# JacobYoung115/VisualSLAM

Measured on AMD Instinct MI355X. Metric: frames/sec @1080p (Harris + DoG keypoint detection), higher is better.
Workload: dtype u8

## Files before the change

visualslam_amd/csrc/kernels_aux.hip.h:

```cpp
#pragma once
#include <hip/hip_runtime.h>

#include "kernels_generic.hip.h"
#include "kernels_localize.hip.h"

namespace vslam {

__global__ __launch_bounds__(256) void k_resize_linear2x_slide(const uint8_t* __restrict__ src, size_t sstep, size_t sframe,
                                                                uint8_t* __restrict__ dst, size_t dframe, int dpitch,
                                                                int rows, int cols, int seg) {
    const int k = blockIdx.x * 256 + threadIdx.x;
    if (4 * k >= cols) return;
    const bool whole = 4 * k + 3 < cols;
    const int m0 = blockIdx.y * seg, m1 = min(m0 + seg, rows);
    const uint8_t* s = src + blockIdx.z * sframe;
    uint8_t* d = dst + blockIdx.z * dframe + 8 * k;
    const int xl = max(4 * k - 1, 0), xr = min(4 * k + 4, cols - 1);
    auto hrow = [&](int m, uint32_t (&X)[4], uint32_t (&Y)[4]) {
        const uint8_t* r = s + (size_t)min(max(m, 0), rows - 1) * sstep;
        uint32_t w;
        if (whole)
            __builtin_memcpy(&w, r + 4 * k, 4);
        else
            w = (uint32_t)r[4 * k] | ((uint32_t)r[min(4 * k + 1, cols - 1)] << 8) | ((uint32_t)r[min(4 * k + 2, cols - 1)] << 16) |
                ((uint32_t)r[cols - 1] << 24);
        const uint32_t s0 = r[xl], s5 = r[xr];
        const uint32_t P = __builtin_amdgcn_perm(w, w, 0x0c010c00);
        const uint32_t Q = __builtin_amdgcn_perm(w, w, 0x0c030c02);
        const uint32_t Qm = __builtin_amdgcn_perm(w, w, 0x0c020c01);
        const uint32_t Pm = s0 | ((w & 0xffu) << 16);
        const uint32_t Qp = (w >> 24) | (s5 << 16);
        const uint32_t P3 = P + (P << 1), Q3 = Q + (Q << 1);
        const uint32_t A[4] = {Pm + P3, P3 + Qm, Qm + Q3, Q3 + Qp};
#pragma unroll
        for (int i = 0; i < 4; ++i) {
            X[i] = pk_lshr_u16(A[i], 2);
            Y[i] = pk_lshr_u16(A[i] + (A[i] << 1), 2);
        }
    };
    auto emit = [&](int dy, const uint32_t (&U)[4], const uint32_t (&V)[4]) {
        uint32_t v[4];
#pragma unroll
        for (int i = 0; i < 4; ++i) v[i] = pk_lshr_u16(U[i] + V[i] + 0x00020002u, 2);
        *reinterpret_cast<uint2*>(d + (size_t)dy * dpitch) = make_uint2(v[0] | (v[1] << 8), v[2] | (v[3] << 8));
    };
    uint32_t Xp[4], Yp[4], Xc[4], Yc[4];
    hrow(m0 - 1, Xp, Yp);
    hrow(m0, Xc, Yc);
    for (int m = m0; m < m1; ++m) {
        uint32_t Xn[4], Yn[4];
        hrow(m + 1, Xn, Yn);
        emit(2 * m, Xp, Yc);
        emit(2 * m + 1, Yc, Xn);
#pragma unroll
        for (int i = 0; i < 4; ++i) Xp[i] = Xc[i], Xc[i] = Xn[i], Yc[i] = Yn[i];
    }
}

__global__ __launch_bounds__(256) void k_resize_nearest_half_v4(const uint8_t* __restrict__ src, size_t sframe, int spitch,
                                                                 uint8_t* __restrict__ dst, size_t dframe, int dpitch,
                                                                 int rows, int drows, int dcols) {
    const int k = blockIdx.x * 256 + threadIdx.x;
    const int y = blockIdx.y;
    if (4 * k >= dcols) return;
    const int sy = min(2 * y, rows - 1);
    const uint2 w = *reinterpret_cast<const uint2*>(src + blockIdx.z * sframe + (size_t)sy * spitch + 8 * k);
    *reinterpret_cast<uint32_t*>(dst + blockIdx.z * dframe + (size_t)y * dpitch + 4 * k) =
        even_bytes(w.x, w.y);
}

constexpr int EXT_SPAN = 768;
constexpr int EXT_PITCH = EXT_SPAN + 16;

template <bool LOC>
__global__ __launch_bounds__(256) void k_extrema_w3(const uint8_t* __restrict__ pyr, size_t pframe, ExtGeom g, int o,
                                                     unsigned long long* __restrict__ bits,
                                                     unsigned long long* __restrict__ lflags, size_t bframe, int li0, int li_step) {
    constexpr int NROW = LOC ? 13 : 10;
    __shared__ __attribute__((aligned(16))) uint8_t srow[NROW * EXT_PITCH + 16];
    __shared__ uint2 queue[LOC ? 768 : 1];
    __shared__ uint8_t qkeep[LOC ? 768 : 1];
    const int li = li0 + (int)blockIdx.y * li_step, f = blockIdx.z;
    const int rows = g.rows[o], cols = g.cols[o], pitch = g.pitch[o];
    const uint32_t P = (uint32_t)rows * (uint32_t)pitch;
    const uint8_t* dog = pyr + f * pframe + g.oct_off[o] + (size_t)VSLAM_NUM_LEVELS * P;
    const int ya = max(3 * li - 1, 0), yb = 3 * li;
    const int yc = min(3 * li + 1, rows - 1);
    const int c0 = blockIdx.x * EXT_SPAN - 16;
    const int wave = __builtin_amdgcn_readfirstlane(threadIdx.x >> 6), lane = threadIdx.x & 63;
    const int cpiece = c0 + 16 * lane;
    const bool piece_ok = lane < EXT_PITCH / 16 && cpiece >= 0 && cpiece < cols;
#pragma unroll
    for (int i = 0; i < (NROW + 3) / 4; ++i) {
        const int rl = wave + 4 * i;
        if (rl < NROW) {
            const int lev = rl < 10 ? (rl >> 1) : rl - 9, y = rl < 10 ? ((rl & 1) ? yb : ya) : yc;
            const uint8_t* rowp = dog + (ptrdiff_t)(int)((uint32_t)lev * P + (uint32_t)y * (uint32_t)pitch + (uint32_t)c0);
            if (piece_ok)
                *reinterpret_cast<uint4*>(srow + rl * EXT_PITCH + 16 * lane) =
                    *reinterpret_cast<const uint4*>(rowp + (uint32_t)(16 * lane));
        }
    }
    if (blockIdx.x == 0 && threadIdx.x < 10)
        srow[threadIdx.x * EXT_PITCH + 15] = dog[(threadIdx.x >> 1) * P + (uint32_t)((threadIdx.x & 1) ? yb : ya) * (uint32_t)pitch];
    __syncthreads();
    const int lc = g.lat_cols[o], wpr = g.wpr[o], lr = g.lat_rows[o];
    const int lj = blockIdx.x * 256 + threadIdx.x;
    bool cand[3] = {false, false, false}, listed[3] = {false, false, false};
    unsigned long long wcand[3], wlist[3];
    const unsigned long long owns = __builtin_amdgcn_ballot_w64(lj < lc);
    const int xa = 3 * (int)threadIdx.x - 1 + 16;
    uint32_t self[5];
    uint32_t up[5], left[5];
    {
        const uint32_t s = xa & 3;
        const uint32_t sel = 0x0c000c00u | s | ((s + 1) << 16);
        uint32_t mn[5], mx[5];
#pragma unroll
        for (int l = 0; l < 5; ++l) {
            uint32_t off = (uint32_t)(xa & ~3) + (uint32_t)(2 * l * EXT_PITCH);
            if (l) asm volatile("" : "+v"(off));
            const uint32_t* q0 = reinterpret_cast<const uint32_t*>(srow + off);
            const uint32_t* q1 = q0 + EXT_PITCH / 4;
            const uint32_t v0 = __builtin_amdgcn_perm(q0[1], q0[0], sel), v1 = __builtin_amdgcn_perm(q1[1], q1[0], sel);
            const uint32_t lo = pk_min_u16(v0, v1), hi = pk_max_u16(v0, v1);
            mn[l] = min(lo & 0xffffu, lo >> 16);
            mx[l] = max(hi & 0xffffu, hi >> 16);
            self[l] = v1 >> 16;
            if (LOC) up[l] = v0 >> 16, left[l] = v1 & 0xffffu;
        }
#pragma unroll
        for (int L = 1; L <= 3; ++L) {
            const uint32_t lo = min(mn[L - 1], min(mn[L], mn[L + 1])), hi = max(mx[L - 1], max(mx[L], mx[L + 1]));
            wcand[L - 1] = (__builtin_amdgcn_ballot_w64(self[L] == lo) | __builtin_amdgcn_ballot_w64(self[L] == hi)) & owns;
            if (LOC) cand[L - 1] = lj < lc && (self[L] == lo || self[L] == hi);
            else wlist[L - 1] = wcand[L - 1] & __builtin_amdgcn_ballot_w64((int)self[L] >= g.min_contrast);
        }
    }
// ... 110 lines not shown
```

visualslam_amd/csrc/vslam_ctx.h:

```cpp
#pragma once
#include <hip/hip_runtime.h>

#include <cstdint>
#include <cstdlib>
#include <deque>
#include <map>
#include <set>
#include <string>
#include <tuple>
#include <utility>
#include <vector>

#include "../../include/vslam.h"

#ifdef VSLAM_DIAGNOSTICS
#define VSLAM_DIAG_ENV(name) std::getenv(name)
#else
#define VSLAM_DIAG_ENV(name) (static_cast<const char*>(nullptr))
#endif

struct StreamTuner {
    static constexpr int K = 3;
    static constexpr int M = K + 1;
    hipStream_t cand[K][2] = {};
    hipEvent_t t0[M] = {}, t1[M] = {};
    int measured = 0;
    int measuring = -1;
    bool enabled = false;
    bool done = false;
    int chosen = 0;
    unsigned long long key = 0;
    int calls = 0, resets = 0;
};

struct JoinWatch {
    static constexpr int RING = 4, NEED = 3;
    hipEvent_t t0[RING] = {}, tm[RING] = {}, t1[RING] = {};
    bool live[RING] = {};
    int head = 0;
    int recording = -1;
    int calls = 0;
    int n_meas = 0;
    float lag[NEED] = {}, best_total = 0.0f;
    float level_best[3] = {0.0f, 0.0f, 0.0f};
    int level = 1;
    int trial_from = -1;
    unsigned long long key = 0;
    int restarts = 0;
    bool done = false, disabled = false, pinned = false;
    float last_lag_frac = -1.0f;
    hipStream_t pair[2][2] = {};
};

struct vslam_ctx {
    int device = 0;
    hipStream_t stream = nullptr;
    bool own_stream = false;
    std::string err;
    char* ws = nullptr;
    size_t ws_cap = 0;
    std::map<std::tuple<int, uint64_t, int>, void*> tables;
    bool mx = false;
    bool f32_fused = false;
    bool orient_scalar_form = false;
    static constexpr int kAux = 3;
    hipStream_t aux[kAux] = {nullptr, nullptr, nullptr};
    hipEvent_t ev_fork = nullptr, ev_join[kAux] = {nullptr, nullptr, nullptr}, ev_oct[VSLAM_MAX_OCTAVES] = {};
    int prio_lo = 0;
    int prio_dev_lo = 0;
    StreamTuner tuner;
    JoinWatch watch;
    hipEvent_t ev_phase = nullptr;
    bool phase_marked = false;
    hipEvent_t ev_up2 = nullptr;
    hipEvent_t ev_chunk = nullptr;
    hipEvent_t ev_pack = nullptr;
    bool pack_pending = false;
    hipEvent_t ev_list0 = nullptr, ev_edge = nullptr;
    hipEvent_t ev_or_fork = nullptr, ev_or_join[2] = {nullptr, nullptr};
    std::vector<std::pair<size_t, void*>> block_cache;
    std::set<const void*> lds_raised;
    float* loc_lut = nullptr;
    uint8_t* dump = nullptr;
    std::string timing_name;
    int launch_tag = -1;
    int timing_tag = -1;
    std::deque<std::pair<hipEvent_t, hipEvent_t>> timing_ev;
    size_t timing_used = 0;
};

static inline int fail(vslam_ctx* c, int code, const std::string& msg) {
    if (c) c->err = msg;
    return code;
}

#define HIPCHK(ctx, expr)                                                                        \
    do {                                                                                         \
        hipError_t e_ = (expr);                                                                  \
        if (e_ != hipSuccess)                                                                    \
            return fail(ctx, e_ == hipErrorOutOfMemory ? VSLAM_ERR_NOMEM : VSLAM_ERR_HIP,        \
                        std::string(#expr) + ": " + hipGetErrorString(e_));                     \
    } while (0)

#define ARGCHK(ctx, cond, msg) \
    if (!(cond)) return fail(ctx, VSLAM_ERR_INVALID, msg)
#define TRY(expr)              \
    do {                       \
        int rc_ = (expr);      \
        if (rc_) return rc_;   \
    } while (0)

static inline int bind_device(vslam_ctx* c) {
    if (!c) return VSLAM_ERR_INVALID;
    HIPCHK(c, hipSetDevice(c->device));
    return VSLAM_OK;
}

namespace vslam {
void sched_init_from_env(vslam_ctx* c);
void sched_destroy(vslam_ctx* c);
int sched_ensure_aux(vslam_ctx* c);
int sched_watch_before_call(vslam_ctx* c, unsigned long long key, bool eligible, bool capturing);
int sched_tuner_before_call(vslam_ctx* c, unsigned long long key, bool eligible);
int sched_tuner_after_call(vslam_ctx* c);
std::pair<hipEvent_t, hipEvent_t>* timing_slot(vslam_ctx* c);
}

struct TimedScope {
    vslam_ctx* c;
    std::pair<hipEvent_t, hipEvent_t>* ev;
    hipStream_t st;
    TimedScope(vslam_ctx* ctx, const char* name, int tag = -1, hipStream_t stream = nullptr)
        : c(ctx), ev(!ctx->timing_name.empty() && ctx->timing_name == name && (ctx->timing_tag < 0 || ctx->timing_tag == tag) ? vslam::timing_slot(ctx) : nullptr),
          st(stream ? stream : ctx->stream) {
        if (ev) (void)hipEventRecord(ev->first, st);
    }
    ~TimedScope() {
        if (ev) (void)hipEventRecord(ev->second, st);
    }
};
```

visualslam_amd/csrc/vslam_hip.hip:

```cpp
#include <hip/hip_runtime.h>

#include <algorithm>
#include <cstdio>
#include <cstdlib>
#include <cstring>
#include <deque>
#include <functional>
#include <map>
#include <string>
#include <set>
#include <memory>
#include <vector>

#include "../../include/vslam.h"
#include "kernels_generic.hip.h"
#include "kernels_pyramid.hip.h"
#include "kernels_strip.hip.h"
#include "kernels_hdiff.hip.h"
#include "kernels_aux.hip.h"
#include "kernels_harris_strip.hip.h"
#include "kernels_orient.hip.h"
#include "kernels_orient_batch.hip.h"
#include "kernels_orient_pk.hip.h"
#include "kernels_compact.hip.h"
// ... 442 lines not shown
}


template <class CFG>
static int enqueue_pyr_octave(vslam_ctx* c, double sigma0, int o, const OctPlan& pl, const OctIO& io) {
    const PyrTaps<CFG>* taps;
    TRY(get_table(c, kTableTile, sigma0, o, "octave kernel", sizeof(PyrTaps<CFG>), [&](void* host) -> int {
        const uint16_t* tp[6];
        tap_pointers(pl.taps, tp);
        pyr_pack_taps<CFG>(tp, *static_cast<PyrTaps<CFG>*>(host));
        return VSLAM_OK;
    }, &taps));
    TRY(raise_dyn_lds(c, reinterpret_cast<const void*>(&k_pyr_octave<CFG>)));
    const dim3 grid((io.cols + CFG::TW - 1) / CFG::TW, (io.rows + CFG::TH - 1) / CFG::TH, io.nf);
    LAUNCH_ON(c, "k_pyr_octave", o, c->stream, CFG::LDS_BYTES, k_pyr_octave<CFG>, grid, dim3(CFG::NT), io.base, io.bframe, io.oct, io.pframe, io.rows,
              io.cols, io.pitch, taps, io.next_base, io.nframe, io.nrows, io.ncols, io.npitch);
    return VSLAM_OK;
}

static int enqueue_pyr_octave_mx(vslam_ctx* c, double sigma0, int o, const OctPlan& pl, const OctIO& io, const MxScan* scan, int up2_step = 0) {
    const void* table;
    TRY(get_table(c, kTableMx, sigma0, o, "matrix-core octave kernel", mx_taps_bytes(pl.mx), [&](void* host) -> int {
        const uint16_t* tp[6];
        tap_pointers(pl.taps, tp);
        if (!mx_pack(pl.mx, tp, host)) return fail(c, VSLAM_ERR_UNSUPPORTED, "matrix-core octave kernel: a tap exceeds 127");
        HIPCHK(c, mx_prepare(pl.mx));
        return VSLAM_OK;
    }, &table));
    hipError_t e;
    {
        TimedScope ts(c, "k_pyr_octave_mx", o);
        e = mx_launch(pl.mx, c->stream, table, io, scan, up2_step);
    }
    HIPCHK(c, e);
    return VSLAM_OK;
}

static int mark_phase(vslam_ctx* c) {
    if (!c->ev_phase) HIPCHK(c, hipEventCreateWithFlags(&c->ev_phase, hipEventDisableTiming));
    HIPCHK(c, hipEventRecord(c->ev_phase, c->stream));
    c->phase_marked = true;
    return VSLAM_OK;
}

static int dog_side_gate(const std::vector<OctPlan>& plans, int nf) {
    int gate = -1;
    if (nf >= 32)
        for (int o = 0; o < (int)plans.size(); ++o)
            if (plans[o].path == OctPath::Tile0 || plans[o].path == OctPath::Tile1) gate = o;
    return gate;
}

static DenseGeom dense_geom(const vslam_batch_layout& L, int o, int min_contrast, int nf) {
    DenseGeom g;
    g.rows = L.rows[o], g.cols = L.cols[o], g.pitch = L.pitch[o];
    g.wpr = (g.cols + 63) / 64;
    g.min_contrast = min_contrast;
    g.P = (unsigned int)((size_t)g.rows * g.pitch);
    g.dog_off = (unsigned int)(L.octave_offset[o] + (size_t)VSLAM_NUM_LEVELS * g.P);
    const long waves_per_rowseg = 4L * (((g.cols + 3) / 4 + 255) / 256) * nf;
    const long segs_wanted = std::max<long>(1, 8192 / waves_per_rowseg);
    g.seg = (int)std::min<long>(XD_SEG_MAX, std::max<long>(4, (g.rows + segs_wanted - 1) / segs_wanted));
    return g;
}

namespace {
struct DogOut {
    uint8_t* pyr;
    size_t pframe;
    unsigned long long* bits = nullptr;
    bool do_extrema = false;
    vslam_point* points = nullptr;
    unsigned int* counts = nullptr;
};

struct DogRun {
    hipStream_t side = nullptr;
    hipStream_t up = nullptr;
    std::function<int(int)> after_list;
    std::function<int(int)> after_octave;
    bool later_chunk = false;
    bool bases_are_scratch = false;
};
}

static int enqueue_octave_scan(vslam_ctx* c, const vslam_params& p, const vslam_batch_layout& L, const ExtGeom& g, const DogScratch& s,
                               const MxScan* fused, int o, int o_done, int nf, const DogOut& out, const DogRun& run) {
    uint8_t* const pyr = out.pyr;
    const size_t pframe = out.pframe;
    unsigned long long* const bits = out.bits;
    const hipStream_t side = run.side;
    if (out.do_extrema && L.lat_rows[o] > 0 && L.lat_cols[o] > 0) {
        hipStream_t es = c->stream;
        if (side) {
            HIPCHK(c, hipStreamWaitEvent(side, c->ev_oct[o_done], 0));
            es = side;
        }
        if (p.extrema_dense) {
            const DenseGeom dg = dense_geom(L, o, p.min_contrast, nf);
            hipLaunchKernelGGL(k_extrema_dense, dim3(((dg.cols + 3) / 4 + 255) / 256, (dg.rows + dg.seg - 1) / dg.seg, nf), dim3(256), 0, es,
                               pyr, pframe, dg, bits ? bits + L.bits_offset[o] : nullptr, s.lflags + L.bits_offset[o], L.bits_frame_words);
        } else if (fused) {
            {
                TimedScope ts(c, "k_extrema_pack", o, es);
                HIPCHK(c, mx_launch_pack(es, *fused, L.rows[o], L.lat_words[o], nf, bits ? bits + L.bits_offset[o] : nullptr, s.lflags + L.bits_offset[o],
                                         L.bits_frame_words, kMxStripRows));
            }
            const int sr = kMxStripRows;
            const int n_straddle = (L.lat_rows[o] - 1) / sr;
            TimedScope ts(c, "k_extrema_w3", o, es);
            if (n_straddle > 0)
                hipLaunchKernelGGL(k_extrema_w3<false>, dim3((L.lat_words[o] + 3) / 4, n_straddle, nf), dim3(256), 0, es, pyr, pframe, g, o, bits, s.lflags,
                                   L.bits_frame_words, sr, sr);
            if (es != c->stream) {
                HIPCHK(c, hipEventRecord(c->ev_pack, es));
                c->pack_pending = true;
            }
        } else if (p.extrema_window == 3) {
            const dim3 eg((L.lat_words[o] + 3) / 4, L.lat_rows[o], nf);
            if (p.localize)
                LAUNCH_ON(c, "k_extrema_w3", o, es, 0, k_extrema_w3<true>, eg, dim3(256), pyr, pframe, g, o, bits, s.lflags, L.bits_frame_words, 0, 1);
            else
                LAUNCH_ON(c, "k_extrema_w3", o, es, 0, k_extrema_w3<false>, eg, dim3(256), pyr, pframe, g, o, bits, s.lflags, L.bits_frame_words, 0, 1);
        } else
            hipLaunchKernelGGL(k_extrema, dim3((L.lat_cols[o] + 255) / 256, L.lat_rows[o], nf * 3), dim3(256), 0, es, pyr,
                               pframe, g, o, bits, s.lflags, L.bits_frame_words);
        HIPCHK(c, hipGetLastError());
    }
    if (out.do_extrema && out.points && out.counts) {
        StreamSwap sw(c, side ? side : c->stream);
        const size_t entries = (size_t)3 * L.lat_rows[o] * L.lat_words[o];
        if (p.extrema_dense) {
            DenseDogEntries ent{s.lflags + L.bits_offset[o], L.bits_frame_words, pyr, pframe, dense_geom(L, o, p.min_contrast, nf), o, out.points};
            TRY(enqueue_compaction(c, ent, entries, nf, s.cws, p.dog_cap, out.counts, o > 0 ? 1 : 0));
        } else {
            DogEntries ent{s.lflags, L.bits_frame_words, pyr, pframe, g, o, o + 1, out.points};
            TRY(enqueue_compaction(c, ent, entries, nf, s.cws, p.dog_cap, out.counts, o > 0 ? 1 : 0));
        }
        if (run.after_list) TRY(run.after_list(o));
    }
    return VSLAM_OK;
}

static int enqueue_dog(vslam_ctx* c, const vslam_params& p, const vslam_batch_layout& L, const std::vector<OctPlan>& plans, const uint8_t* frames,
                       size_t fstep, size_t fframe, int nf, DogScratch& s, const DogOut& out, const DogRun& run = DogRun()) {
    const hipStream_t side = run.side, up = run.up;
    const int gate = (side && p.localize) ? dog_side_gate(plans, nf) : -1;
    ExtGeom g;
    if (p.localize) TRY(ensure_loc_lut(c));
    fill_geom(c, p, L, g);
    const bool up2_fused = c->mx && run.bases_are_scratch && L.n_octaves > 0 && L.rows[0] == 2 * p.rows && L.cols[0] == 2 * p.cols && fstep <= 0x7fffffff &&
                           mx_up2_supported(plans[0].mx);
    const int nf_a = (!up2_fused && side && up && nf >= 64) ? nf / 2 : nf;
    if (!up2_fused)
        LAUNCH(c, "k_resize_linear2x_slide", k_resize_linear2x_slide, dim3(((p.cols + 3) / 4 + 255) / 256, (p.rows + 15) / 16, nf_a), dim3(256),
               frames, fstep, fframe, s.bases + s.base_off[0], s.bases_frame, L.pitch[0], p.rows, p.cols, 16);
    if (nf_a < nf) {
        if (run.later_chunk) HIPCHK(c, hipStreamWaitEvent(up, c->ev_chunk, 0));
        StreamSwap sw(c, up);
        LAUNCH(c, "k_resize_linear2x_slide", k_resize_linear2x_slide, dim3(((p.cols + 3) / 4 + 255) / 256, (p.rows + 15) / 16, nf - nf_a), dim3(256),
               frames + (size_t)nf_a * fframe, fstep, fframe, s.bases + s.base_off[0] + (size_t)nf_a * s.bases_frame, s.bases_frame, L.pitch[0],
               p.rows, p.cols, 16);
        HIPCHK(c, hipEventRecord(c->ev_up2, c->stream));
    }
    bool fused[VSLAM_MAX_OCTAVES] = {};
    if (run.later_chunk && c->pack_pending) {
        HIPCHK(c, hipStreamWaitEvent(c->stream, c->ev_pack, 0));
        c->pack_pending = false;
    }
    MxScan scan[VSLAM_MAX_OCTAVES] = {};
    struct TagReset {
        vslam_ctx* c;
        ~TagReset() { c->launch_tag = -1; }
    } tag_reset{c};
    for (int o = 0; o < L.n_octaves; ++o) {
        c->launch_tag = o;
        const int rows = L.rows[o], cols = L.cols[o], pitch = L.pitch[o];
        const size_t P = (size_t)rows * pitch;
        const OctPlan& pl = plans[o];
        const bool has_next = o + 1 < L.n_octaves;
        const bool fuse_next = has_next && pl.path != OctPath::Generic;
        OctIO io{s.bases + s.base_off[o], s.bases_frame, out.pyr + L.octave_offset[o], out.pframe, rows, cols, pitch, nf,
                 fuse_next ? s.bases + s.base_off[o + 1] : nullptr, s.bases_frame, has_next ? L.rows[o + 1] : 0, has_next ? L.cols[o + 1] : 0,
                 has_next ? L.pitch[o + 1] : 0};
        if (o == 0 && up2_fused) io.base = frames, io.bframe = fframe;
        const int shape = (long)((cols + 255) / 256) * ((rows + 31) / 32) <= (long)((cols + 127) / 128) * ((rows + 63) / 64) ? 1 : 0;
        fused[o] = c->mx && s.sitemap && out.do_extrema && !p.localize && !p.extrema_dense && p.extrema_window == 3 && L.lat_rows[o] > 0 &&
                   L.lat_cols[o] > 0 && mx_scan_supported(pl.mx);
        if (fused[o])
            scan[o] = MxScan{s.sitemap + s.site_off[o], s.site_frame, L.lat_rows[o], L.lat_cols[o], s.site_pitch[o], p.min_contrast,
                             s.colmap + s.col_off[o], s.col_frame, mx_seams(cols)};
        auto tiled = [&](int f_lo, int n) -> int {
            const OctIO part = io.frames(f_lo, n);
            if (c->mx && pl.mx) {
                MxScan sc = scan[o];
                if (fused[o]) sc.sitemap += (size_t)f_lo * s.site_frame, sc.colmap += (size_t)f_lo * s.col_frame;
                return enqueue_pyr_octave_mx(c, p.sigma0, o, pl, part, fused[o] ? &sc : nullptr, o == 0 && up2_fused ? (int)fstep : 0);
            }
            if (pl.path == OctPath::Tile0)
                return shape == 1 ? enqueue_pyr_octave<PyrCfgOct0W>(c, p.sigma0, o, pl, part) : enqueue_pyr_octave<PyrCfgOct0>(c, p.sigma0, o, pl, part);
            return shape == 1 ? enqueue_pyr_octave<PyrCfgOct1W>(c, p.sigma0, o, pl, part) : enqueue_pyr_octave<PyrCfgOct1>(c, p.sigma0, o, pl, part);
        };
        const bool is_tiled = pl.path == OctPath::Tile0 || pl.path == OctPath::Tile1 || (c->mx && pl.mx != 0);
        if (o == 0 && nf_a < nf && !is_tiled) HIPCHK(c, hipStreamWaitEvent(c->stream, c->ev_up2, 0));
        if (is_tiled && o == 0 && nf_a < nf) {
            TRY(tiled(0, nf_a));
            HIPCHK(c, hipStreamWaitEvent(c->stream, c->ev_up2, 0));
            TRY(tiled(nf_a, nf - nf_a));
        } else if (is_tiled)
            TRY(tiled(0, nf));
        else if (pl.path == OctPath::Strip)
            TRY(enqueue_strip_octave(c, p.sigma0, o, pl, io, s.h));
        else {
            for (int l = 0; l < VSLAM_NUM_LEVELS; ++l)
                TRY(enqueue_blur(c, io.base, (size_t)pitch, s.bases_frame, io.oct + (size_t)l * P, (size_t)pitch, out.pframe, s.h, rows,
                                 cols, nf, pl.ks[l], pl.sg[l]));
            LAUNCH(c, "k_dog5", k_dog5, dim3((unsigned)((P + 255) / 256), 1, nf), dim3(256), io.oct,
                   io.oct + (size_t)VSLAM_NUM_LEVELS * P, P, out.pframe);
        }
        if (has_next && !fuse_next)
            LAUNCH(c, "k_resize_nearest_half_v4", k_resize_nearest_half_v4, dim3((L.cols[o + 1] / 4 + 256) / 256, L.rows[o + 1], nf),
                   dim3(256), io.oct + (size_t)3 * P, out.pframe, pitch, s.bases + s.base_off[o + 1], s.bases_frame, L.pitch[o + 1], rows,
                   L.rows[o + 1], L.cols[o + 1]);
        if (side) HIPCHK(c, hipEventRecord(c->ev_oct[o], c->stream));
        if (o == 0) TRY(mark_phase(c));
        if (run.after_octave) TRY(run.after_octave(o));
        if (o < gate) continue;
        for (int oo = (o == gate ? 0 : o); oo <= o; ++oo) TRY(enqueue_octave_scan(c, p, L, g, s, fused[oo] ? &scan[oo] : nullptr, oo, o, nf, out, run));
    }
    if (side && up) HIPCHK(c, hipEventRecord(c->ev_chunk, c->stream));
    return VSLAM_OK;
}

static size_t harris_flag_words(int rows, int cols) { return (size_t)rows * ((cols + HS_STRIP_W - 1) / HS_STRIP_W) * 4; }

static int enqueue_harris(vslam_ctx* c, const uint8_t* frames, size_t fframe, int rows, int cols, int nf, float k,
                          float* resp, uint8_t* mask, float* nms2, unsigned long long* hflags, vslam_kp* kps,
                          unsigned int cap, unsigned int* counts, unsigned int* chunk_ws) {
    const size_t N = (size_t)rows * cols;
    if (N >= ((size_t)1 << 31)) return fail(c, VSLAM_ERR_UNSUPPORTED, "Harris: images of 2^31 pixels or more are not supported (32-bit row offsets)");
    const bool aligned = cols % 4 == 0 && fframe % 4 == 0;
    HarrisStripArgs a;
    a.img = frames;
    a.frame = fframe;
    a.rows = rows;
    a.cols = cols;
    a.k = k;
    a.resp = resp;
    a.mask = mask;
    a.nms2 = nms2;
    a.flags = hflags;
    a.nstrips = (cols + HS_STRIP_W - 1) / HS_STRIP_W;
    a.fframe = (size_t)rows * a.nstrips * 4;
    if (!c->dump) HIPCHK(c, hipMalloc((void**)&c->dump, 256));
    a.dump = c->dump;
    const long want_seg = std::max<long>(1, 12288 / ((long)a.nstrips * nf));
    a.seg = (int)std::min<long>(rows, std::max<long>(16, (rows + want_seg - 1) / want_seg));
    const int nseg = (rows + a.seg - 1) / a.seg;
    if (aligned)
        LAUNCH(c, "k_harris_strip", k_harris_strip<false>, dim3((a.nstrips * nseg + 3) / 4, 1, nf), dim3(256), a);
    else
        LAUNCH(c, "k_harris_strip", k_harris_strip<true>, dim3((a.nstrips * nseg + 3) / 4, 1, nf), dim3(256), a);
    if (hflags && kps && counts) {
        HarrisStripEntries ent{hflags, a.fframe, rows, cols, a.nstrips, resp, N, kps};
        TRY(enqueue_compaction(c, ent, (size_t)rows * a.nstrips, nf, chunk_ws, cap, counts, 0));
    }
    return VSLAM_OK;
}

static int h2d(vslam_ctx* c, void* dst, size_t dpitch, const void* src, size_t spitch, size_t width_bytes,
               size_t rows) {
    if (dpitch == width_bytes && spitch == width_bytes)
        HIPCHK(c, hipMemcpyAsync(dst, src, width_bytes * rows, hipMemcpyHostToDevice, c->stream));
    else
        HIPCHK(c, hipMemcpy2DAsync(dst, dpitch, src, spitch, width_bytes, rows, hipMemcpyHostToDevice, c->stream));
    return VSLAM_OK;
}
static int d2h(vslam_ctx* c, void* dst, size_t dpitch, const void* src, size_t spitch, size_t width_bytes,
               size_t rows) {
    if (dpitch == width_bytes && spitch == width_bytes)
        HIPCHK(c, hipMemcpyAsync(dst, src, width_bytes * rows, hipMemcpyDeviceToHost, c->stream));
    else
        HIPCHK(c, hipMemcpy2DAsync(dst, dpitch, src, spitch, width_bytes, rows, hipMemcpyDeviceToHost, c->stream));
    return VSLAM_OK;
}

template <class R>
static int read_list(vslam_ctx* c, const unsigned int* d_count, const R* d_list, size_t cap, R* out, size_t* count, uint64_t* bits = nullptr,
                     const unsigned long long* d_bits = nullptr, size_t bits_bytes = 0) {
    unsigned int n = 0;
    HIPCHK(c, hipMemcpyAsync(&n, d_count, 4, hipMemcpyDeviceToHost, c->stream));
    if (bits_bytes) HIPCHK(c, hipMemcpyAsync(bits, d_bits, bits_bytes, hipMemcpyDeviceToHost, c->stream));
    TRY(vslam_ctx_sync(c));
    *count = n;
    const size_t m = std::min<size_t>(n, cap);
    if (m) HIPCHK(c, hipMemcpy(out, d_list, m * sizeof(R), hipMemcpyDeviceToHost));
    return VSLAM_OK;
}


extern "C" {


int vslam_ctx_create(int device, void* stream, vslam_ctx** out) {
    if (!out || device < 0) return VSLAM_ERR_INVALID;
    *out = nullptr;
    int n = 0;
    if (hipGetDeviceCount(&n) != hipSuccess || device >= n) return VSLAM_ERR_HIP;
    if (hipSetDevice(device) != hipSuccess) return VSLAM_ERR_HIP;
    vslam_ctx* c = new (std::nothrow) vslam_ctx();
    if (!c) return VSLAM_ERR_NOMEM;
    c->device = device;
    if (stream == VSLAM_STREAM_LEGACY) {
        c->stream = nullptr;
    } else if (stream) {
        c->stream = (hipStream_t)stream;
    } else {
        if (hipStreamCreateWithFlags(&c->stream, hipStreamNonBlocking) != hipSuccess) {
            delete c;
            return VSLAM_ERR_HIP;
        }
        c->own_stream = true;
    }
    {
        const char* e = std::getenv("VSLAM_MX");
        c->mx = e && e[0] == '1';
        const char* ff = std::getenv("VSLAM_F32_FUSED");
        c->f32_fused = ff && ff[0] == '1';
        const char* es = VSLAM_DIAG_ENV("VSLAM_ORIENT_SCALAR");
        c->orient_scalar_form = es && es[0] == '1';
        sched_init_from_env(c);
    }
    *out = c;
    return VSLAM_OK;
}

int vslam_ctx_set_matrix_path(vslam_ctx* c, int on) {
    if (!c) return VSLAM_ERR_INVALID;
    c->mx = on != 0;
    return VSLAM_OK;
}

int vslam_ctx_get_matrix_path(const vslam_ctx* c) { return c && c->mx ? 1 : 0; }

int vslam_ctx_set_f32_fused(vslam_ctx* c, int on) {
    if (!c) return VSLAM_ERR_INVALID;
    c->f32_fused = on != 0;
    return VSLAM_OK;
}

int vslam_ctx_get_f32_fused(const vslam_ctx* c) { return c && c->f32_fused ? 1 : 0; }

int vslam_ctx_destroy(vslam_ctx* c) {
    if (!c) return VSLAM_ERR_INVALID;
    (void)hipSetDevice(c->device);
    (void)hipStreamSynchronize(c->stream);
    for (int i = 0; i < vslam_ctx::kAux; ++i)
        if (c->aux[i]) (void)hipStreamSynchronize(c->aux[i]);
    for (auto& kv : c->tables) (void)hipFree(kv.second);
    if (c->ws) (void)hipFree(c->ws);
    for (auto& b : c->block_cache) (void)hipFree(b.second);
    if (c->loc_lut) (void)hipFree(c->loc_lut);
    if (c->dump) (void)hipFree(c->dump);
    sched_destroy(c);
    for (hipEvent_t e : {c->ev_phase, c->ev_up2, c->ev_chunk, c->ev_pack, c->ev_list0, c->ev_edge, c->ev_or_fork, c->ev_or_join[0], c->ev_or_join[1]})
        if (e) (void)hipEventDestroy(e);
    for (auto& e : c->ev_oct)
        if (e) (void)hipEventDestroy(e);
    if (c->own_stream) (void)hipStreamDestroy(c->stream);
    delete c;
    return VSLAM_OK;
}

int vslam_ctx_sync(vslam_ctx* c) {
    TRY(bind_device(c));
    HIPCHK(c, hipStreamSynchronize(c->stream));
    return VSLAM_OK;
}

const char* vslam_last_error(const vslam_ctx* c) { return c ? c->err.c_str() : "null context"; }
const char* vslam_kernel_names(void) { return kKernelNames; }



int vslam_gaussian_blur_u8(vslam_ctx* c, const uint8_t* src, int rows, int cols, size_t step, int ksize,
                           double sigma, uint8_t* dst, size_t dst_step) {
    TRY(bind_device(c));
    ARGCHK(c, src && dst && rows > 0 && cols > 0 && step >= (size_t)cols && dst_step >= (size_t)cols, "blur: bad image");
    const int n = ksize > 0 ? ksize : (sigma > 0 ? gauss_ksize_u8(sigma) : -1);
    ARGCHK(c, n > 0 && (n & 1) && n <= VSLAM_MAX_KSIZE, "blur: kernel size must be odd (or 0 with sigma > 0)");
    const size_t P = (size_t)rows * cols;
    uint8_t *d_src, *d_dst;
    uint16_t* d_h;
    WsPlan ws;
    ws.add(d_src, P), ws.add(d_dst, P), ws.add(d_h, P);
    TRY(ws.commit(c));
    TRY(h2d(c, d_src, cols, src, step, cols, rows));
    TRY(enqueue_blur(c, d_src, cols, P, d_dst, cols, P, d_h, rows, cols, 1, n, sigma));
    TRY(d2h(c, dst, dst_step, d_dst, cols, cols, rows));
    return vslam_ctx_sync(c);
}

int vslam_sobel_k1_u8_f32(vslam_ctx* c, const uint8_t* src, int rows, int cols, size_t step, int dx, int dy,
                          float* dst, size_t dst_step) {
    TRY(bind_device(c));
    ARGCHK(c, src && dst && rows > 0 && cols > 0 && step >= (size_t)cols && dst_step >= 4 * (size_t)cols, "sobel: bad image");
    ARGCHK(c, (dx == 1 && dy == 0) || (dx == 0 && dy == 1), "sobel: (dx,dy) must be (1,0) or (0,1)");
    const size_t P = (size_t)rows * cols;
    uint8_t* d_src;
    float* d_dst;
    WsPlan ws;
    ws.add(d_src, P), ws.add(d_dst, P);
    TRY(ws.commit(c));
    TRY(h2d(c, d_src, cols, src, step, cols, rows));
    LAUNCH(c, "k_sobel_k1", k_sobel_k1, grid_rows(cols, rows), dim3(256), d_src, (size_t)cols, d_dst, (size_t)cols, rows,
           cols, dx);
    TRY(d2h(c, dst, dst_step, d_dst, 4 * (size_t)cols, 4 * (size_t)cols, rows));
    return vslam_ctx_sync(c);
}

int vslam_resize_linear2x_u8(vslam_ctx* c, const uint8_t* src, int rows, int cols, size_t step, uint8_t* dst,
                             size_t dst_step) {
    TRY(bind_device(c));
    ARGCHK(c, src && dst && rows > 0 && cols > 0 && step >= (size_t)cols && dst_step >= 2 * (size_t)cols, "resize2x: bad image");
    const size_t P = (size_t)rows * cols;
    uint8_t *d_src, *d_dst;
    WsPlan ws;
    ws.add(d_src, P), ws.add(d_dst, 4 * P);
    TRY(ws.commit(c));
    TRY(h2d(c, d_src, cols, src, step, cols, rows));
    if (cols % 4 == 0)
        LAUNCH(c, "k_resize_linear2x_slide", k_resize_linear2x_slide, dim3((cols / 4 + 255) / 256, (rows + 15) / 16, 1), dim3(256),
               d_src, (size_t)cols, P, d_dst, 4 * P, 2 * cols, rows, cols, 16);
    else
        LAUNCH(c, "k_resize_linear2x", k_resize_linear2x, grid_rows(2 * cols, 2 * rows), dim3(256), d_src, (size_t)cols, P,
               d_dst, (size_t)2 * cols, 4 * P, rows, cols);
    TRY(d2h(c, dst, dst_step, d_dst, 2 * (size_t)cols, 2 * (size_t)cols, 2 * (size_t)rows));
    return vslam_ctx_sync(c);
}

int vslam_resize_nearest_half_u8(vslam_ctx* c, const uint8_t* src, int rows, int cols, size_t step, uint8_t* dst,
                                 size_t dst_step) {
    TRY(bind_device(c));
    int dr, dc;
    half_size(rows, cols, &dr, &dc);
    ARGCHK(c, src && dst && rows > 0 && cols > 0 && dr > 0 && dc > 0 && step >= (size_t)cols && dst_step >= (size_t)dc,
           "resize half: bad image");
    const size_t P = (size_t)rows * cols, Q = (size_t)dr * dc;
    uint8_t *d_src, *d_dst;
    WsPlan ws;
    ws.add(d_src, P), ws.add(d_dst, Q);
    TRY(ws.commit(c));
    TRY(h2d(c, d_src, cols, src, step, cols, rows));
    LAUNCH(c, "k_resize_nearest_half", k_resize_nearest_half, grid_rows(dc, dr), dim3(256), d_src, (size_t)cols, P, d_dst,
           (size_t)dc, Q, rows, cols, dr, dc);
    TRY(d2h(c, dst, dst_step, d_dst, dc, dc, dr));
    return vslam_ctx_sync(c);
}

int vslam_convert_scale_abs_f32(vslam_ctx* c, const float* src, int rows, int cols, size_t step, uint8_t* dst,
                                size_t dst_step) {
    TRY(bind_device(c));
    ARGCHK(c, src && dst && rows > 0 && cols > 0 && step >= 4 * (size_t)cols && dst_step >= (size_t)cols, "convertScaleAbs: bad image");
    const size_t P = (size_t)rows * cols;
    float* d_src;
    uint8_t* d_dst;
    WsPlan ws;
    ws.add(d_src, P), ws.add(d_dst, P);
    TRY(ws.commit(c));
    TRY(h2d(c, d_src, 4 * (size_t)cols, src, step, 4 * (size_t)cols, rows));
    LAUNCH(c, "k_convert_scale_abs", k_convert_scale_abs, grid_rows(cols, rows), dim3(256), d_src, (size_t)cols, d_dst,
           (size_t)cols, rows, cols);
    TRY(d2h(c, dst, dst_step, d_dst, cols, cols, rows));
    return vslam_ctx_sync(c);
}


int vslam_harris_from_grad_f32(vslam_ctx* c, const float* ix, const float* iy, int rows, int cols, size_t step,
                               float k, int window, float* resp, size_t resp_step) {
    TRY(bind_device(c));
    ARGCHK(c, ix && iy && resp && rows > 0 && cols > 0 && step >= 4 * (size_t)cols && resp_step >= 4 * (size_t)cols,
           "HarrisCorner: bad image");
    ARGCHK(c, window >= 1 && (window & 1), "HarrisCorner: window must be odd");
    const size_t P = (size_t)rows * cols, rb = 4 * (size_t)cols;
    float *d_ix, *d_iy, *d_r;
    WsPlan ws;
    ws.add(d_ix, P), ws.add(d_iy, P), ws.add(d_r, P);
    TRY(ws.commit(c));
    TRY(h2d(c, d_ix, rb, ix, step, rb, rows));
    TRY(h2d(c, d_iy, rb, iy, step, rb, rows));
    LAUNCH(c, "k_harris_from_grad", k_harris_from_grad, grid_rows(cols, rows), dim3(256), d_ix, d_iy, (size_t)cols, rows,
           cols, k, (window - 1) / 2, d_r, (size_t)cols);
    TRY(d2h(c, resp, resp_step, d_r, rb, rb, rows));
    return vslam_ctx_sync(c);
}

int vslam_harris_response_u8(vslam_ctx* c, const uint8_t* img, int rows, int cols, size_t step, float k, int window,
                             float* resp, size_t resp_step) {
    TRY(bind_device(c));
    ARGCHK(c, img && resp && rows > 0 && cols > 0 && step >= (size_t)cols && resp_step >= 4 * (size_t)cols,
           "harris_response: bad image");
    if (window != 3) return fail(c, VSLAM_ERR_UNSUPPORTED, "harris_response: fused kernel implements windowSize 3 (Harris_corners.cpp:34); use the per-stage entry points for other windows");
    const size_t P = (size_t)rows * cols;
    uint8_t* d_img;
    float* d_r;
    WsPlan ws;
    ws.add(d_img, P), ws.add(d_r, P);
    TRY(ws.commit(c));
    TRY(h2d(c, d_img, cols, img, step, cols, rows));
    TRY(enqueue_harris(c, d_img, P, rows, cols, 1, k, d_r, nullptr, nullptr, nullptr, nullptr, 0, nullptr, nullptr));
    TRY(d2h(c, resp, resp_step, d_r, 4 * (size_t)cols, 4 * (size_t)cols, rows));
    return vslam_ctx_sync(c);
}

static int nms_strict_common(vslam_ctx* c, const void* src, int elem, int rows, int cols, size_t step, int window,
                             uint8_t* mask, size_t mask_step) {
// ... 941 lines not shown
```

visualslam_amd/csrc/vslam_sched.cpp:

```cpp
#include "vslam_ctx.h"

#include <algorithm>

namespace vslam {

std::pair<hipEvent_t, hipEvent_t>* timing_slot(vslam_ctx* c) {
    if (c->timing_used == c->timing_ev.size()) {
        if (c->timing_ev.size() >= 65536) return nullptr;
        hipEvent_t a, b;
        if (hipEventCreate(&a) != hipSuccess) return nullptr;
        if (hipEventCreate(&b) != hipSuccess) {
            (void)hipEventDestroy(a);
            return nullptr;
        }
        c->timing_ev.emplace_back(a, b);
    }
    return &c->timing_ev[c->timing_used++];
}

static int tuner_pair_of(int slot) { return slot == StreamTuner::K ? 0 : slot; }

static int create_side_stream(vslam_ctx* c, int prio_lo, hipStream_t* out) {
    if (prio_lo == 0 || hipStreamCreateWithPriority(out, hipStreamNonBlocking, prio_lo) != hipSuccess) {
        (void)hipGetLastError();
// ... 118 lines not shown
            w.trial_from = -1;
            w.done = true;
            return VSLAM_OK;
        }
        w.key = key;
    }
    if (w.level <= 1 && !w.pair[w.level][0]) w.pair[w.level][0] = c->aux[0], w.pair[w.level][1] = c->aux[1];
    for (int i = 0; i < JoinWatch::RING; ++i) {
        if (!w.live[i]) continue;
        const hipError_t q = hipEventQuery(w.t1[i]);
        if (q == hipErrorNotReady) {
            (void)hipGetLastError();
            continue;
        }
        w.live[i] = false;
        float total = 0.0f, lag = 0.0f;
        if (q != hipSuccess || hipEventElapsedTime(&total, w.t0[i], w.t1[i]) != hipSuccess || hipEventElapsedTime(&lag, w.tm[i], w.t1[i]) != hipSuccess || !(total > 0.0f)) {
            (void)hipGetLastError();
            continue;
        }
        w.last_lag_frac = lag / total;
        if (w.n_meas < JoinWatch::NEED) {
            w.lag[w.n_meas++] = lag / total;
            w.best_total = (w.best_total == 0.0f || total < w.best_total) ? total : w.best_total;
        }
    }
    if (w.n_meas >= JoinWatch::NEED) {
        const float a = w.lag[0], b = w.lag[1], m = w.lag[2];
        const float med = std::max(std::min(a, b), std::min(std::max(a, b), m));
        w.level_best[w.level] = w.best_total;
        bool keep = true;
        if (w.trial_from >= 0 && !(w.best_total < 0.99f * w.level_best[w.trial_from])) {
            TRY(watch_set_level(c, w.trial_from));
            w.trial_from = -1;
            w.done = true;
            keep = false;
        }
        if (keep) {
            w.trial_from = -1;
            const float limit = w.level == 0 ? 0.03f : 0.10f;
            if (w.level < 2 && med > limit && (w.level == 1 || c->prio_dev_lo != 0)) {
                const int from = w.level;
                TRY(watch_set_level(c, from + 1));
                w.trial_from = from;
            } else
                w.done = true;
        }
        if (w.done) return VSLAM_OK;
    }
    if (!eligible) return VSLAM_OK;
    if (++w.calls == 1) return VSLAM_OK;
    const int slot = w.head;
    if (w.live[slot]) return VSLAM_OK;
    if (!w.t0[slot]) {
        HIPCHK(c, hipEventCreate(&w.t0[slot]));
        HIPCHK(c, hipEventCreate(&w.tm[slot]));
        HIPCHK(c, hipEventCreate(&w.t1[slot]));
    }
    HIPCHK(c, hipEventRecord(w.t0[slot], c->stream));
    w.recording = slot;
    w.head = (slot + 1) % JoinWatch::RING;
    return VSLAM_OK;
}

int sched_ensure_aux(vslam_ctx* c) {
    if (c->ev_fork) return VSLAM_OK;
    int prio_lo = 0, prio_hi = 0;
    if (hipDeviceGetStreamPriorityRange(&prio_lo, &prio_hi) != hipSuccess) {
        (void)hipGetLastError();
        prio_lo = 0;
    }
    c->prio_dev_lo = prio_lo;
    if (prio_lo == 0 && c->watch.level == 0) c->watch.level = 1;
    c->prio_lo = c->watch.level >= 1 ? 0 : prio_lo;
    for (int i = 0; i < vslam_ctx::kAux; ++i) {
        if (i == 2)
            HIPCHK(c, hipStreamCreateWithFlags(&c->aux[i], hipStreamNonBlocking));
        else
            TRY(create_side_stream(c, c->prio_lo, &c->aux[i]));
        HIPCHK(c, hipEventCreateWithFlags(&c->ev_join[i], hipEventDisableTiming));
    }
    c->tuner.cand[0][0] = c->aux[0], c->tuner.cand[0][1] = c->aux[1];
    for (auto& e : c->ev_oct) HIPCHK(c, hipEventCreateWithFlags(&e, hipEventDisableTiming));
    HIPCHK(c, hipEventCreateWithFlags(&c->ev_up2, hipEventDisableTiming));
    HIPCHK(c, hipEventCreateWithFlags(&c->ev_chunk, hipEventDisableTiming));
    HIPCHK(c, hipEventCreateWithFlags(&c->ev_pack, hipEventDisableTiming));
    HIPCHK(c, hipEventCreateWithFlags(&c->ev_list0, hipEventDisableTiming));
    HIPCHK(c, hipEventCreateWithFlags(&c->ev_edge, hipEventDisableTiming));
    HIPCHK(c, hipEventCreateWithFlags(&c->ev_or_fork, hipEventDisableTiming));
    for (auto& e : c->ev_or_join) HIPCHK(c, hipEventCreateWithFlags(&e, hipEventDisableTiming));
    HIPCHK(c, hipEventCreateWithFlags(&c->ev_fork, hipEventDisableTiming));
    return VSLAM_OK;
}

void sched_init_from_env(vslam_ctx* c) {
    const char* jw = std::getenv("VSLAM_JOIN_WATCH");
    c->watch.disabled = jw && jw[0] == '0';
    if (const char* sp = std::getenv("VSLAM_SIDE_PRIORITY")) c->watch.level = (sp[0] == 'l' || sp[0] == 'L') ? 0 : 1;
    const char* t = std::getenv("VSLAM_STREAM_TUNER");
    if (t && t[0] == '1') (void)vslam_ctx_tune_side_streams(c, 1);
}

void sched_destroy(vslam_ctx* c) {
    for (auto& ev : c->timing_ev) {
        (void)hipEventDestroy(ev.first);
        (void)hipEventDestroy(ev.second);
    }
    if (c->ev_fork && !c->tuner.done) tuner_finish(c, 0);
    for (int i = 0; i < vslam_ctx::kAux; ++i) {
        if (c->aux[i]) (void)hipStreamDestroy(c->aux[i]);
        if (c->ev_join[i]) (void)hipEventDestroy(c->ev_join[i]);
    }
    if (c->ev_fork) (void)hipEventDestroy(c->ev_fork);
    for (int i = 0; i < JoinWatch::RING; ++i)
        for (hipEvent_t e : {c->watch.t0[i], c->watch.tm[i], c->watch.t1[i]})
            if (e) (void)hipEventDestroy(e);
    for (auto& pr : c->watch.pair)
        for (hipStream_t st : pr)
            if (st && st != c->aux[0] && st != c->aux[1]) (void)hipStreamSynchronize(st), (void)hipStreamDestroy(st);
}

}

using namespace vslam;

extern "C" {

int vslam_kernel_timing_enable(vslam_ctx* c, const char* name) {
    if (!c) return VSLAM_ERR_INVALID;
    c->timing_name = name ? name : "";
    c->timing_tag = -1;
    const size_t at = c->timing_name.find('@');
    if (at != std::string::npos) {
        c->timing_tag = std::atoi(c->timing_name.c_str() + at + 1);
        c->timing_name.resize(at);
    }
    c->timing_used = 0;
    return VSLAM_OK;
}
int vslam_kernel_timing_read(vslam_ctx* c, int* launches, double* total_ms) {
    TRY(bind_device(c));
    HIPCHK(c, hipStreamSynchronize(c->stream));
    double tot = 0;
    for (size_t i = 0; i < c->timing_used; ++i) {
        float ms = 0;
        HIPCHK(c, hipEventElapsedTime(&ms, c->timing_ev[i].first, c->timing_ev[i].second));
        tot += ms;
    }
    if (launches) *launches = (int)c->timing_used;
    if (total_ms) *total_ms = tot;
    c->timing_used = 0;
    return VSLAM_OK;
}

int vslam_ctx_side_stream_report(const vslam_ctx* c, int* pair, int* state) {
    if (!c) return VSLAM_ERR_INVALID;
    if (pair) *pair = c->tuner.chosen;
    if (state) *state = c->tuner.done ? 2 : ((c->tuner.enabled && c->tuner.calls > 1) ? 1 : 0);
    return VSLAM_OK;
}

int vslam_ctx_set_side_stream_priority(vslam_ctx* c, int low) {
    if (!c) return VSLAM_ERR_INVALID;
    if (c->ev_fork) return fail(c, VSLAM_ERR_UNSUPPORTED, "set_side_stream_priority: the side streams exist already - call it before the context's first batch call");
    if (!c->watch.pinned) c->watch.level = low ? 0 : 1;
    return VSLAM_OK;
}
// ... 35 lines not shown
```

Before: 14800.

## Rework 2x upsample kernel with DPP neighbours and split head into three stream parts

The linear 2x upsample kernel now loads all rows of its 16-row segment up front and obtains horizontal neighbour pixels through DPP lane shifts instead of extra byte loads. It also replaces the shift-and-round steps with fused shift/mask and byte-permute packing. On the host, the upsample head is split into up to three frame chunks on a side stream, each with its own event, so the tiled octave-0 pass can begin on earlier chunks sooner. The cost is more registers from the unrolled segment arrays, plus extra launches and stream waits.

```diff
diff --git a/visualslam_amd/csrc/kernels_aux.hip.h b/visualslam_amd/csrc/kernels_aux.hip.h
--- a/visualslam_amd/csrc/kernels_aux.hip.h
+++ b/visualslam_amd/csrc/kernels_aux.hip.h
@@ -6,54 +6,68 @@
 
 namespace vslam {
 
+constexpr int UP_SEG = 16;
 __global__ __launch_bounds__(256) void k_resize_linear2x_slide(const uint8_t* __restrict__ src, size_t sstep, size_t sframe,
                                                                 uint8_t* __restrict__ dst, size_t dframe, int dpitch,
-                                                                int rows, int cols, int seg) {
-    const int k = blockIdx.x * 256 + threadIdx.x;
-    if (4 * k >= cols) return;
+                                                                int rows, int cols) {
+    const int k = blockIdx.x * 256 + threadIdx.x, lane = threadIdx.x & 63;
+    if (4 * (k - lane) >= cols) return;
+    const bool inside = 4 * k < cols;
     const bool whole = 4 * k + 3 < cols;
-    const int m0 = blockIdx.y * seg, m1 = min(m0 + seg, rows);
+    const int m0 = blockIdx.y * UP_SEG;
     const uint8_t* s = src + blockIdx.z * sframe;
-    uint8_t* d = dst + blockIdx.z * dframe + 8 * k;
-    const int xl = max(4 * k - 1, 0), xr = min(4 * k + 4, cols - 1);
-    auto hrow = [&](int m, uint32_t (&X)[4], uint32_t (&Y)[4]) {
-        const uint8_t* r = s + (size_t)min(max(m, 0), rows - 1) * sstep;
-        uint32_t w;
+    uint8_t* d = dst + blockIdx.z * dframe + (size_t)(2 * m0) * dpitch;
+    const int c0 = min(4 * k, cols - 1), c1 = min(4 * k + 1, cols - 1), c2 = min(4 * k + 2, cols - 1), c3 = min(4 * k + 3, cols - 1);
+    const bool edge = lane == 0 || lane == 63;
+    const int ce = lane == 0 ? max(c0 - 1, 0) : min(4 * k + 4, cols - 1);
+    const uint32_t sel_pm = lane == 0 ? 0x0c000c04u : 0x0c000c07u;
+    uint32_t W[UP_SEG + 2], E[UP_SEG + 2];
+#pragma unroll
+    for (int i = 0; i < UP_SEG + 2; ++i) {
+        const uint8_t* r = s + (size_t)min(max(m0 - 1 + i, 0), rows - 1) * sstep;
         if (whole)
-            __builtin_memcpy(&w, r + 4 * k, 4);
+            __builtin_memcpy(&W[i], r + 4 * k, 4);
+        else if (!inside)
+            W[i] = r[cols - 1];
         else
-            w = (uint32_t)r[4 * k] | ((uint32_t)r[min(4 * k + 1, cols - 1)] << 8) | ((uint32_t)r[min(4 * k + 2, cols - 1)] << 16) |
-                ((uint32_t)r[cols - 1] << 24);
-        const uint32_t s0 = r[xl], s5 = r[xr];
+            W[i] = (uint32_t)r[c0] | ((uint32_t)r[c1] << 8) | ((uint32_t)r[c2] << 16) | ((uint32_t)r[c3] << 24);
+        E[i] = 0;
+        if (edge) E[i] = r[ce];
+    }
+    auto hrow = [&](int i, uint32_t (&X)[4], uint32_t (&Y)[4]) {
+        const uint32_t w = W[i], e = E[i];
+        const uint32_t wl = __builtin_amdgcn_update_dpp(e, w, 0x138, 0xf, 0xf, false);
+        const uint32_t wr = __builtin_amdgcn_update_dpp(e, w, 0x130, 0xf, 0xf, false);
         const uint32_t P = __builtin_amdgcn_perm(w, w, 0x0c010c00);
         const uint32_t Q = __builtin_amdgcn_perm(w, w, 0x0c030c02);
         const uint32_t Qm = __builtin_amdgcn_perm(w, w, 0x0c020c01);
-        const uint32_t Pm = s0 | ((w & 0xffu) << 16);
-        const uint32_t Qp = (w >> 24) | (s5 << 16);
+        const uint32_t Pm = __builtin_amdgcn_perm(wl, w, sel_pm);
+        const uint32_t Qp = __builtin_amdgcn_perm(wr, w, 0x0c040c03);
         const uint32_t P3 = P + (P << 1), Q3 = Q + (Q << 1);
         const uint32_t A[4] = {Pm + P3, P3 + Qm, Qm + Q3, Q3 + Qp};
 #pragma unroll
-        for (int i = 0; i < 4; ++i) {
-            X[i] = pk_lshr_u16(A[i], 2);
-            Y[i] = pk_lshr_u16(A[i] + (A[i] << 1), 2);
+        for (int j = 0; j < 4; ++j) {
+            const uint32_t T = A[j] << 4;
+            X[j] = T & 0xffc0ffc0u;
+            asm("v_lshl_add_u32 %0, %1, 1, %1" : "=v"(Y[j]) : "v"(T));
         }
     };
     auto emit = [&](int dy, const uint32_t (&U)[4], const uint32_t (&V)[4]) {
-        uint32_t v[4];
-#pragma unroll
-        for (int i = 0; i < 4; ++i) v[i] = pk_lshr_u16(U[i] + V[i] + 0x00020002u, 2);
-        *reinterpret_cast<uint2*>(d + (size_t)dy * dpitch) = make_uint2(v[0] | (v[1] << 8), v[2] | (v[3] << 8));
+        uint32_t t[4];
+#pragma unroll
+        for (int j = 0; j < 4; ++j) t[j] = U[j] + V[j] + 0x00800080u;
+        if (inside && m0 + (dy >> 1) < rows)
+            *reinterpret_cast<uint2*>(d + (size_t)dy * dpitch + (uint32_t)(8 * k)) =
+                make_uint2(__builtin_amdgcn_perm(t[1], t[0], 0x07030501), __builtin_amdgcn_perm(t[3], t[2], 0x07030501));
     };
-    uint32_t Xp[4], Yp[4], Xc[4], Yc[4];
-    hrow(m0 - 1, Xp, Yp);
-    hrow(m0, Xc, Yc);
-    for (int m = m0; m < m1; ++m) {
-        uint32_t Xn[4], Yn[4];
-        hrow(m + 1, Xn, Yn);
-        emit(2 * m, Xp, Yc);
-        emit(2 * m + 1, Yc, Xn);
-#pragma unroll
-        for (int i = 0; i < 4; ++i) Xp[i] = Xc[i], Xc[i] = Xn[i], Yc[i] = Yn[i];
+    uint32_t X[UP_SEG + 2][4], Y[UP_SEG + 2][4];
+    hrow(0, X[0], Y[0]);
+    hrow(1, X[1], Y[1]);
+#pragma unroll
+    for (int i = 0; i < UP_SEG; ++i) {
+        hrow(i + 2, X[i + 2], Y[i + 2]);
+        emit(2 * i, X[i], Y[i + 1]);
+        emit(2 * i + 1, Y[i + 1], X[i + 2]);
     }
 }
 
diff --git a/visualslam_amd/csrc/vslam_ctx.h b/visualslam_amd/csrc/vslam_ctx.h
--- a/visualslam_amd/csrc/vslam_ctx.h
+++ b/visualslam_amd/csrc/vslam_ctx.h
@@ -72,7 +72,8 @@
     JoinWatch watch;
     hipEvent_t ev_phase = nullptr;
     bool phase_marked = false;
-    hipEvent_t ev_up2 = nullptr;
+    static constexpr int kHeadParts = 3;
+    hipEvent_t ev_up[kHeadParts - 1] = {};
     hipEvent_t ev_chunk = nullptr;
     hipEvent_t ev_pack = nullptr;
     bool pack_pending = false;
diff --git a/visualslam_amd/csrc/vslam_hip.hip b/visualslam_amd/csrc/vslam_hip.hip
--- a/visualslam_amd/csrc/vslam_hip.hip
+++ b/visualslam_amd/csrc/vslam_hip.hip
@@ -548,6 +548,19 @@
     bool later_chunk = false;
     bool bases_are_scratch = false;
 };
+
+constexpr int kHeadCum8[vslam_ctx::kHeadParts] = {4, 8, 8};
+constexpr int kHeadMinFrames = 32;
+int head_parts(int nf, int (&n)[vslam_ctx::kHeadParts]) {
+    int cnt = 0;
+    for (int i = 0, lo = 0; i < vslam_ctx::kHeadParts && lo < nf; ++i) {
+        int hi = std::max((nf * kHeadCum8[i] + 4) / 8, lo + kHeadMinFrames);
+        if (i + 1 == vslam_ctx::kHeadParts || nf - hi < kHeadMinFrames) hi = nf;
+        n[cnt++] = hi - lo;
+        lo = hi;
+    }
+    return cnt;
+}
 }
 
 static int enqueue_octave_scan(vslam_ctx* c, const vslam_params& p, const vslam_batch_layout& L, const ExtGeom& g, const DogScratch& s,
@@ -617,17 +630,22 @@
     fill_geom(c, p, L, g);
     const bool up2_fused = c->mx && run.bases_are_scratch && L.n_octaves > 0 && L.rows[0] == 2 * p.rows && L.cols[0] == 2 * p.cols && fstep <= 0x7fffffff &&
                            mx_up2_supported(plans[0].mx);
-    const int nf_a = (!up2_fused && side && up && nf >= 64) ? nf / 2 : nf;
-    if (!up2_fused)
-        LAUNCH(c, "k_resize_linear2x_slide", k_resize_linear2x_slide, dim3(((p.cols + 3) / 4 + 255) / 256, (p.rows + 15) / 16, nf_a), dim3(256),
-               frames, fstep, fframe, s.bases + s.base_off[0], s.bases_frame, L.pitch[0], p.rows, p.cols, 16);
-    if (nf_a < nf) {
+    int head_n[vslam_ctx::kHeadParts] = {nf};
+    const int n_head = (!up2_fused && side && up && nf >= 2 * kHeadMinFrames) ? head_parts(nf, head_n) : 1;
+    auto upsample = [&](int f_lo, int n) -> int {
+        LAUNCH(c, "k_resize_linear2x_slide", k_resize_linear2x_slide, dim3(((p.cols + 3) / 4 + 255) / 256, (p.rows + UP_SEG - 1) / UP_SEG, n), dim3(256),
+               frames + (size_t)f_lo * fframe, fstep, fframe, s.bases + s.base_off[0] + (size_t)f_lo * s.bases_frame, s.bases_frame, L.pitch[0],
+               p.rows, p.cols);
+        return VSLAM_OK;
+    };
+    if (!up2_fused) TRY(upsample(0, head_n[0]));
+    if (n_head > 1) {
         if (run.later_chunk) HIPCHK(c, hipStreamWaitEvent(up, c->ev_chunk, 0));
         StreamSwap sw(c, up);
-        LAUNCH(c, "k_resize_linear2x_slide", k_resize_linear2x_slide, dim3(((p.cols + 3) / 4 + 255) / 256, (p.rows + 15) / 16, nf - nf_a), dim3(256),
-               frames + (size_t)nf_a * fframe, fstep, fframe, s.bases + s.base_off[0] + (size_t)nf_a * s.bases_frame, s.bases_frame, L.pitch[0],
-               p.rows, p.cols, 16);
-        HIPCHK(c, hipEventRecord(c->ev_up2, c->stream));
+        for (int i = 1, f_lo = head_n[0]; i < n_head; f_lo += head_n[i++]) {
+            TRY(upsample(f_lo, head_n[i]));
+            HIPCHK(c, hipEventRecord(c->ev_up[i - 1], c->stream));
+        }
     }
     bool fused[VSLAM_MAX_OCTAVES] = {};
     if (run.later_chunk && c->pack_pending) {
@@ -668,11 +686,13 @@
             return shape == 1 ? enqueue_pyr_octave<PyrCfgOct1W>(c, p.sigma0, o, pl, part) : enqueue_pyr_octave<PyrCfgOct1>(c, p.sigma0, o, pl, part);
         };
         const bool is_tiled = pl.path == OctPath::Tile0 || pl.path == OctPath::Tile1 || (c->mx && pl.mx != 0);
-        if (o == 0 && nf_a < nf && !is_tiled) HIPCHK(c, hipStreamWaitEvent(c->stream, c->ev_up2, 0));
-        if (is_tiled && o == 0 && nf_a < nf) {
-            TRY(tiled(0, nf_a));
-            HIPCHK(c, hipStreamWaitEvent(c->stream, c->ev_up2, 0));
-            TRY(tiled(nf_a, nf - nf_a));
+        if (o == 0 && !is_tiled)
+            for (int i = 1; i < n_head; ++i) HIPCHK(c, hipStreamWaitEvent(c->stream, c->ev_up[i - 1], 0));
+        if (is_tiled && o == 0 && n_head > 1) {
+            for (int i = 0, f_lo = 0; i < n_head; f_lo += head_n[i++]) {
+                if (i > 0) HIPCHK(c, hipStreamWaitEvent(c->stream, c->ev_up[i - 1], 0));
+                TRY(tiled(f_lo, head_n[i]));
+            }
         } else if (is_tiled)
             TRY(tiled(0, nf));
         else if (pl.path == OctPath::Strip)
@@ -829,7 +849,9 @@
     if (c->loc_lut) (void)hipFree(c->loc_lut);
     if (c->dump) (void)hipFree(c->dump);
     sched_destroy(c);
-    for (hipEvent_t e : {c->ev_phase, c->ev_up2, c->ev_chunk, c->ev_pack, c->ev_list0, c->ev_edge, c->ev_or_fork, c->ev_or_join[0], c->ev_or_join[1]})
+    for (hipEvent_t e : {c->ev_phase, c->ev_chunk, c->ev_pack, c->ev_list0, c->ev_edge, c->ev_or_fork, c->ev_or_join[0], c->ev_or_join[1]})
+        if (e) (void)hipEventDestroy(e);
+    for (auto& e : c->ev_up)
         if (e) (void)hipEventDestroy(e);
     for (auto& e : c->ev_oct)
         if (e) (void)hipEventDestroy(e);
@@ -896,8 +918,8 @@
     TRY(ws.commit(c));
     TRY(h2d(c, d_src, cols, src, step, cols, rows));
     if (cols % 4 == 0)
-        LAUNCH(c, "k_resize_linear2x_slide", k_resize_linear2x_slide, dim3((cols / 4 + 255) / 256, (rows + 15) / 16, 1), dim3(256),
-               d_src, (size_t)cols, P, d_dst, 4 * P, 2 * cols, rows, cols, 16);
+        LAUNCH(c, "k_resize_linear2x_slide", k_resize_linear2x_slide, dim3((cols / 4 + 255) / 256, (rows + UP_SEG - 1) / UP_SEG, 1), dim3(256),
+               d_src, (size_t)cols, P, d_dst, 4 * P, 2 * cols, rows, cols);
     else
         LAUNCH(c, "k_resize_linear2x", k_resize_linear2x, grid_rows(2 * cols, 2 * rows), dim3(256), d_src, (size_t)cols, P,
                d_dst, (size_t)2 * cols, 4 * P, rows, cols);
diff --git a/visualslam_amd/csrc/vslam_sched.cpp b/visualslam_amd/csrc/vslam_sched.cpp
--- a/visualslam_amd/csrc/vslam_sched.cpp
+++ b/visualslam_amd/csrc/vslam_sched.cpp
@@ -224,7 +224,7 @@
     }
     c->tuner.cand[0][0] = c->aux[0], c->tuner.cand[0][1] = c->aux[1];
     for (auto& e : c->ev_oct) HIPCHK(c, hipEventCreateWithFlags(&e, hipEventDisableTiming));
-    HIPCHK(c, hipEventCreateWithFlags(&c->ev_up2, hipEventDisableTiming));
+    for (auto& e : c->ev_up) HIPCHK(c, hipEventCreateWithFlags(&e, hipEventDisableTiming));
     HIPCHK(c, hipEventCreateWithFlags(&c->ev_chunk, hipEventDisableTiming));
     HIPCHK(c, hipEventCreateWithFlags(&c->ev_pack, hipEventDisableTiming));
     HIPCHK(c, hipEventCreateWithFlags(&c->ev_list0, hipEventDisableTiming));
```

Result: no change. 14800 (median of 3 runs) (-0.0%).
